# lars-frogner/Impact

Measured on AMD Instinct MI355X. Metric: voxels stepped/sec + remesh tris/sec, 512^3 grid, 1/2/4/8 MI355X, higher is better.
Workload: dtype i8 voxels, f32 SDF/mesh arithmetic, f64 moments; 1 GPU; config-2 SDF asteroid x2.05 -> 502^3 grid = 512^3 stored voxels (32768 chunks); parallelism=single GPU, voxels_per_gpu=134217728, regions=1, triangles=1813104

## Files before the change

### impact_amd/csrc/derive.hip

```cpp
#include "chunk_passes.hpp"
#include "table_roles.hpp"
#include "many.hpp"

#ifndef IVX_DERIVE_WAVES
#define IVX_DERIVE_WAVES 6
#endif

namespace {

struct DeriveParams {
    uint32_t cx, cy, cz;
};

__device__ __forceinline__ uint32_t row_mask(uint4 s) {
    uint32_t w[4] = {s.x, s.y, s.z, s.w};
    uint32_t m = 0;
#pragma unroll
    for (int q = 0; q < 4; ++q) m |= ((((w[q] >> 7) & 0x01010101u) * 0x00204081u >> 21) & 0xFu) << (4 * q);
    return m;
}

__device__ __forceinline__ uint32_t nbr_row_mask(const GridView& g, const ivx_chunk_info* info, size_t c, uint32_t off) {
    const uint32_t gen = info[c].gen_kind;
    const uint32_t rm = row_mask(*reinterpret_cast<const uint4*>(g.sdf + c * IVX_CHUNK_VOXELS + off));
// ... 465 lines not shown
            const bool only_empty = (cnt[0] | cnt[1] | cnt[2] | cnt[3] | cnt[4] | cnt[5]) == 0 && (ci_.flags & CF_ONLY_EMPTY);
            ci_.flags = (uint8_t)(ob | (only_empty ? CF_ONLY_EMPTY : 0u));
            uint32_t fd = 0;
#pragma unroll
            for (int f = 0; f < 6; ++f) fd |= own_fd[f] << (2 * f);
            ci_.face_dist = (uint16_t)fd;
            ci_.uniform_type = 0;
        } else if (kind == KIND_UNIFORM) {
            ci_.flags = 0;
            ci_.face_dist = 0x555;
            ci_.uniform_type = (uint8_t)utype;
        } else {
            ci_.flags = 0;
            ci_.face_dist = 0;
        }
        info[chunk] = ci_;
    }
    IVX_T(g, li, 5);
    }
}
template <bool SIGNS>
__global__ __launch_bounds__(256) __attribute__((amdgpu_waves_per_eu(IVX_DERIVE_WAVES, 8))) void k_derive(DeriveArgs a) {
    derive_body<SIGNS>(a, blockIdx.x, gridDim.x);
}
IVX_MANY_TWIN(k_derive_planes_many, DeriveArgs, derive_body<false>, __launch_bounds__(256) __attribute__((amdgpu_waves_per_eu(IVX_DERIVE_WAVES, 8))))
IVX_MANY_TWIN(k_derive_signs_many, DeriveArgs, derive_body<true>, __launch_bounds__(256) __attribute__((amdgpu_waves_per_eu(IVX_DERIVE_WAVES, 8))))
IVX_MANY_LAUNCHER(many_derive_planes, k_derive_planes_many, DeriveArgs, 256)
IVX_MANY_LAUNCHER(many_derive_signs, k_derive_signs_many, DeriveArgs, 256)

#ifndef IVX_DERIVE_FLOOD_CAP
#define IVX_DERIVE_FLOOD_CAP 32
#endif
#ifndef IVX_DERIVE_WAVE_WAVES
#define IVX_DERIVE_WAVE_WAVES 5
#endif

#ifdef IVX_WG_TRACE
#define IVX_TW(g, entry, slot)                                                                      \
    do {                                                                                            \
        if ((threadIdx.x & 63u) == 0u) (g).trace[(size_t)(entry) * 8 + (slot)] = wall_clock64();    \
    } while (0)
#else
#define IVX_TW(g, entry, slot) \
    do {                       \
    } while (0)
#endif

__device__ __forceinline__ void ivx_wave_lds_sync() {
    __builtin_amdgcn_fence(__ATOMIC_SEQ_CST, "workgroup");
    __builtin_amdgcn_wave_barrier();
}
__device__ __forceinline__ uint32_t ivx_run_fill_up(uint32_t m, uint32_t x) { return m & (((m + x) ^ m) | x); }
__device__ __forceinline__ uint32_t ivx_run_fill(uint32_t m, uint32_t x) {
    x &= m;
    return ivx_run_fill_up(m, x) | __builtin_bitreverse32(ivx_run_fill_up(__builtin_bitreverse32(m), __builtin_bitreverse32(x)));
}
__device__ __forceinline__ uint32_t ivx_dpp_u32_shr1(uint32_t v) { return (uint32_t)__builtin_amdgcn_update_dpp(0, (int)v, 0x111, 0xF, 0xF, true); }
__device__ __forceinline__ uint32_t ivx_dpp_u32_shl1(uint32_t v) { return (uint32_t)__builtin_amdgcn_update_dpp(0, (int)v, 0x101, 0xF, 0xF, true); }
__device__ __forceinline__ uint32_t ivx_wave_or(uint32_t v) {
    v |= (uint32_t)__builtin_amdgcn_update_dpp(0, (int)v, 0x111, 0xF, 0xF, true);
    v |= (uint32_t)__builtin_amdgcn_update_dpp(0, (int)v, 0x112, 0xF, 0xF, true);
    v |= (uint32_t)__builtin_amdgcn_update_dpp(0, (int)v, 0x114, 0xF, 0xF, true);
    v |= (uint32_t)__builtin_amdgcn_update_dpp(0, (int)v, 0x118, 0xF, 0xF, true);
    return ((uint32_t)__builtin_amdgcn_readlane((int)v, 15) | (uint32_t)__builtin_amdgcn_readlane((int)v, 31)) |
           ((uint32_t)__builtin_amdgcn_readlane((int)v, 47) | (uint32_t)__builtin_amdgcn_readlane((int)v, 63));
}

// ... 20 lines not shown
            G |= q > 0 ? F[q > 0 ? q - 1 : 0] : (a > 0u ? up : 0u);
            G |= q < 3 ? F[q < 3 ? q + 1 : 3] : (a < 3u ? dn : 0u);
            N[q] = ivx_run_fill(M[q], G);
            miss = miss || N[q] != M[q];
            grew = grew || N[q] != F[q];
        }
        if (!__ballot(miss)) return 1u;
        if (!__ballot(grew)) return 0u;
#pragma unroll
        for (int q = 0; q < 4; ++q) F[q] = N[q];
    }
    return 0u;
}

__device__ __forceinline__ void moments_rows_wave(double D, double Dz1, double Dz2, double (*s_red)[10], uint32_t i, uint32_t j, int gi, int gj) {
    const double I = (double)gi, J = (double)gj;
    const double qx = 2.0 * I + 1.0, qy = 2.0 * J + 1.0;
    const double cx = 3.0 * I * I + 3.0 * I + 1.0, cy = 3.0 * J * J + 3.0 * J + 1.0;
    const double r0 = ivx_row16_sum_f64(D), r1 = ivx_row16_sum_f64(D * qy), r2 = ivx_row16_sum_f64(D * cy);
    const double r3 = ivx_row16_sum_f64(Dz1), r4 = ivx_row16_sum_f64(qy * Dz1), r5 = ivx_row16_sum_f64(Dz2);
    if (j == 15u) {
        double* o = s_red[i];
        o[0] = r0;
        o[1] = r0 * qx;
        o[2] = r1;
        o[3] = r3;
        o[4] = r2 + r5;
        o[5] = r0 * cx + r5;
        o[6] = r0 * cx + r2;
        o[7] = r1 * qx;
        o[8] = r4;
        o[9] = r3 * qx;
    }
}

__device__ __forceinline__ void derive_wave_body(const DeriveArgs& a_) {
    const GridView& g = a_.g;
    uint8_t* __restrict__ flags_out = a_.flags_out;
    int8_t* __restrict__ sdf_rw = a_.sdf_rw;
    uint8_t* __restrict__ type_rw = a_.type_rw;
    ivx_chunk_info* __restrict__ info = a_.info;
    uint16_t* __restrict__ signs = a_.signs;
    uint8_t* __restrict__ kface_out = a_.kface_out;
    uint32_t* __restrict__ active_list = a_.active_list;
    const uint32_t* __restrict__ list_in = a_.list_in;
    const DeriveFused& fz = a_.fz;
    __shared__ float s_dens[256];
    __shared__ uint16_t s_mtab[256];
    __shared__ uint16_t s_occ[4][18 * 18 + 4];
    __shared__ double s_red_all[4][16][10];
    const uint32_t tid = threadIdx.x, lane = tid & 63u;
    const uint32_t wave = (uint32_t)__builtin_amdgcn_readfirstlane((int)(tid >> 6));
    uint16_t* occ = s_occ[wave];
    double (*s_red)[10] = s_red_all[wave];
    if (fz.parts & IVX_PART_MOMENTS) s_dens[tid] = fz.dens[tid], s_mtab[tid] = moments_table_entry(tid);
    __syncthreads();
    const uint32_t la = lane >> 4, j = lane & 15u;
    const uint32_t n_active = a_.work_counts[0];
    const uint32_t n_walk = gridDim.x * 4u;
    const uint32_t sx = g.cy * g.cz;
    const uint32_t* sw = reinterpret_cast<const uint32_t*>(g.signs);
    for (uint32_t li = ivx_xcd_remap(blockIdx.x, gridDim.x) * 4u + wave; li < n_active; li += n_walk) {
    IVX_TW(g, li, 0);
    const uint32_t chunk = IVX_LIST_CHUNK(list_in[li]);
    const int ck = chunk % g.cz, cj = (chunk / g.cz) % g.cy, ci = chunk / sx;
    const size_t base = (size_t)chunk * IVX_CHUNK_VOXELS;
    const bool has_zlo = ck > 0, has_zhi = ck + 1 < (int)g.cz;
    const size_t c_lo = has_zlo ? (size_t)chunk - 1 : (size_t)chunk, c_hi = has_zhi ? (size_t)chunk + 1 : (size_t)chunk;
    const uint32_t nf = la, nr = j;
    bool n_present;
    size_t nc;
    uint32_t noff;
    if (nf == 0) n_present = ci > 0, nc = (size_t)chunk - sx, noff = 240u + nr;
    else if (nf == 1) n_present = ci + 1 < (int)g.cx, nc = (size_t)chunk + sx, noff = nr;
    else if (nf == 2) n_present = cj > 0, nc = (size_t)chunk - g.cz, noff = nr * 16u + 15u;
    else n_present = cj + 1 < (int)g.cy, nc = (size_t)chunk + g.cz, noff = nr * 16u;
    if (!n_present) nc = chunk;
    uint2 own_rec = reinterpret_cast<const uint2*>(info)[chunk];
    uint32_t gen_lo = reinterpret_cast<const uint32_t*>(info)[2 * c_lo], gen_hi = reinterpret_cast<const uint32_t*>(info)[2 * c_hi];
    uint32_t ngen = reinterpret_cast<const uint32_t*>(info)[2 * nc];
    uint32_t type0 = *reinterpret_cast<const uint32_t*>(g.type + base);
    uint32_t nrow = sw[(nc * 256 + noff) >> 1];
    uint32_t ow[4], bl[4], bh[4];
#pragma unroll
    for (int q = 0; q < 4; ++q) {
        const uint32_t r = (4u * la + q) * 16u + j;
        ow[q] = sw[((size_t)chunk * 256 + r) >> 1];
        bl[q] = sw[(c_lo * 256 + r) >> 1];
        bh[q] = sw[(c_hi * 256 + r) >> 1];
    }
    asm volatile("" : "+v"(own_rec.x), "+v"(own_rec.y), "+v"(gen_lo), "+v"(gen_hi), "+v"(ngen), "+v"(type0), "+v"(nrow));
    asm volatile("" : "+v"(ow[0]), "+v"(ow[1]), "+v"(ow[2]), "+v"(ow[3]), "+v"(bl[0]), "+v"(bl[1]), "+v"(bl[2]), "+v"(bl[3]));
    asm volatile("" : "+v"(bh[0]), "+v"(bh[1]), "+v"(bh[2]), "+v"(bh[3]));
    own_rec.x = (uint32_t)__builtin_amdgcn_readfirstlane((int)own_rec.x), own_rec.y = (uint32_t)__builtin_amdgcn_readfirstlane((int)own_rec.y);
    gen_lo = ((uint32_t)__builtin_amdgcn_readfirstlane((int)gen_lo) >> 8) & 0xFFu, gen_hi = ((uint32_t)__builtin_amdgcn_readfirstlane((int)gen_hi) >> 8) & 0xFFu;
    type0 = (uint32_t)__builtin_amdgcn_readfirstlane((int)type0);
    ngen = (ngen >> 8) & 0xFFu;
    ivx_chunk_info own_info;
    own_info.kind = (uint8_t)(own_rec.x & 0xFFu);
    own_info.gen_kind = (uint8_t)((own_rec.x >> 8) & 0xFFu);
    own_info.flags = (uint8_t)((own_rec.x >> 16) & 0xFFu);
    own_info.uniform_type = (uint8_t)(own_rec.x >> 24);
    own_info.face_dist = (uint16_t)(own_rec.y & 0xFFFFu);
    own_info.region_count = (uint8_t)((own_rec.y >> 16) & 0xFFu);
    own_info.boundary_region_count = (uint8_t)(own_rec.y >> 24);
    const uint32_t gen = own_info.gen_kind;
    const bool own_uniform = gen == KIND_UNIFORM;
    uint32_t m[4], zl = 0u, zh = 0u;
    const uint32_t half = 16u * (j & 1u);
#pragma unroll
    for (int q = 0; q < 4; ++q) {
        m[q] = own_uniform ? 0xFFFFu : (gen == KIND_VOID ? 0u : ((ow[q] >> half) & 0xFFFFu));
        const uint32_t lo = (bl[q] >> half >> 15) & 1u, hi = (bh[q] >> half) & 1u;
        if (has_zlo && (gen_lo == KIND_NONUNIFORM ? lo : (gen_lo == KIND_UNIFORM ? 1u : 0u))) zl |= 1u << q;
        if (has_zhi && (gen_hi == KIND_NONUNIFORM ? hi : (gen_hi == KIND_UNIFORM ? 1u : 0u))) zh |= 1u << q;
        occ[(4u * la + q + 1u) * 18u + j + 1u] = (uint16_t)m[q];
    }
    uint32_t nm = 0u;
    {
        const uint32_t nrow_odd = nf == 2 ? 1u : (nf == 3 ? 0u : (nr & 1u));
        const uint32_t rm = (nrow >> (16u * nrow_odd)) & 0xFFFFu;
        if (n_present) nm = ngen == KIND_NONUNIFORM ? rm : (ngen == KIND_UNIFORM ? 0xFFFFu : 0u);
        if (nf == 0) occ[0 * 18 + nr + 1] = (uint16_t)nm;
        else if (nf == 1) occ[17 * 18 + nr + 1] = (uint16_t)nm;
        else if (nf == 2) occ[(nr + 1) * 18 + 0] = (uint16_t)nm;
        else occ[(nr + 1) * 18 + 17] = (uint16_t)nm;
    }
    uint32_t cnt[12];
    {
        const uint32_t p0 = __popc(m[0]), p3 = __popc(m[3]), pc = (p0 + __popc(m[1])) + (__popc(m[2]) + p3);
        cnt[0] = (uint32_t)__builtin_amdgcn_readlane((int)ivx_row16_sum(p0), 15);
        cnt[1] = (uint32_t)__builtin_amdgcn_readlane((int)ivx_row16_sum(p3), 63);
        cnt[2] = ((uint32_t)__builtin_amdgcn_readlane((int)pc, 0) + (uint32_t)__builtin_amdgcn_readlane((int)pc, 16)) +
                 ((uint32_t)__builtin_amdgcn_readlane((int)pc, 32) + (uint32_t)__builtin_amdgcn_readlane((int)pc, 48));
        cnt[3] = ((uint32_t)__builtin_amdgcn_readlane((int)pc, 15) + (uint32_t)__builtin_amdgcn_readlane((int)pc, 31)) +
                 ((uint32_t)__builtin_amdgcn_readlane((int)pc, 47) + (uint32_t)__builtin_amdgcn_readlane((int)pc, 63));
        uint32_t z0 = 0, z1 = 0, nz0 = 0, nz1 = 0;
#pragma unroll
        for (int q = 0; q < 4; ++q) {
            z0 += (uint32_t)__popcll(__ballot((m[q] & 1u) != 0u));
            z1 += (uint32_t)__popcll(__ballot(((m[q] >> 15) & 1u) != 0u));
            nz0 += (uint32_t)__popcll(__ballot(((zl >> q) & 1u) != 0u));
            nz1 += (uint32_t)__popcll(__ballot(((zh >> q) & 1u) != 0u));
        }
        cnt[4] = z0, cnt[5] = z1, cnt[10] = nz0, cnt[11] = nz1;
        const uint32_t nfs = ivx_row16_sum(__popc(nm));
        cnt[6] = (uint32_t)__builtin_amdgcn_readlane((int)nfs, 15), cnt[7] = (uint32_t)__builtin_amdgcn_readlane((int)nfs, 31);
        cnt[8] = (uint32_t)__builtin_amdgcn_readlane((int)nfs, 47), cnt[9] = (uint32_t)__builtin_amdgcn_readlane((int)nfs, 63);
    }
    {
        uint32_t bi = 0, bjw = 0;
#pragma unroll
        for (int q = 0; q < 4; ++q) {
            const unsigned long long b = __ballot(m[q] != 0u);
#pragma unroll
            for (int s = 0; s < 4; ++s)
                if ((b >> (16 * s)) & 0xFFFFull) bi |= 1u << (4 * s + q);
            bjw |= (uint32_t)b | (uint32_t)(b >> 32);
        }
        const uint32_t bj = (bjw | (bjw >> 16)) & 0xFFFFu;
        const uint32_t ku = ivx_wave_or((m[0] | m[1]) | (m[2] | m[3]));
        uint32_t packed = 0;
        if (bi) {
            packed = 0x80000000u | (uint32_t)(__ffs(bi) - 1) | ((uint32_t)(31 - __clz(bi)) << 4) | ((uint32_t)(__ffs(bj) - 1) << 8) |
                     ((uint32_t)(31 - __clz(bj)) << 12) | ((uint32_t)(__ffs(ku) - 1) << 16) | ((uint32_t)(31 - __clz(ku)) << 20);
        }
        if (lane == 0u && IVX_DBG_KEEP(64u)) a_.bbox[chunk] = packed;
    }
    IVX_TW(g, li, 1);
    uint32_t own_fd[6], nbr_full = 0, own_mixed = 0;
#pragma unroll
    for (int f = 0; f < 6; ++f) {
        const uint32_t c = cnt[f];
        own_fd[f] = c == 0 ? FD_EMPTY : (c == 256 ? FD_FULL : FD_MIXED);
        if (own_fd[f] == FD_MIXED) own_mixed |= 1u << f;
        if (cnt[6 + f] == 256) nbr_full |= 1u << f;
    }
    uint32_t kind = gen;
    if (gen == KIND_UNIFORM && nbr_full != 0x3Fu) kind = KIND_NONUNIFORM;
    const uint32_t utype = own_uniform ? (own_info.kind == KIND_NONUNIFORM ? (type0 & 0xFFu) : (uint32_t)own_info.uniform_type) : 0u;
    const bool fresh = own_uniform && own_info.kind != KIND_NONUNIFORM;
    const uint32_t quirk = own_mixed & nbr_full;
    ivx_wave_lds_sync();
    IVX_TW(g, li, 2);
    bool t_x = false, t_y = false, t_z = false;
#pragma unroll
    for (int q = 0; q < 4; ++q) {
        const uint32_t i = 4u * la + q, r = i * 16u + j;
        const uint32_t xdn = occ[i * 18u + j + 1u], xup = occ[(i + 2u) * 18u + j + 1u];
        const uint32_t ydn = occ[(i + 1u) * 18u + j], yup = occ[(i + 1u) * 18u + j + 2u];
        const uint32_t mq = m[q], zlo = (zl >> q) & 1u, zhi = (zh >> q) & 1u;
        t_x = t_x || (i == 15u && (mq & xup) != 0u);
        t_y = t_y || (j == 15u && (mq & yup) != 0u);
        t_z = t_z || ((((mq >> 15) & 1u) & zhi) != 0u);
        if (kind != KIND_NONUNIFORM) continue;
        const uint32_t zdn = (mq << 1) | zlo, zup = (mq >> 1) | (zhi << 15);
        const uint32_t e = ~mq & 0xFFFFu;
        uint32_t dm[6];
        dm[0] = (mq & xdn) | ((i == 0u && (quirk & 1u)) ? e : 0u);
        dm[1] = (mq & ydn) | ((j == 0u && (quirk & 4u)) ? e : 0u);
// ... 57 lines not shown
            }
            all_full = !__ballot(not_full);
            any = __ballot(nonempty) != 0ull;
            touches = __ballot(on_edge) != 0ull;
            const bool several_runs = __ballot(runs2) != 0ull;
            const uint32_t lack_all = ivx_wave_or(lack);
            if (any && !all_full && !several_runs && (~lack_all & 0xFFFFu) != 0u) {
                uint32_t b[16];
#pragma unroll
                for (int q = 0; q < 4; ++q) {
                    const unsigned long long bq = __ballot(R[q] != 0u);
#pragma unroll
                    for (int s = 0; s < 4; ++s) b[4 * s + q] = (uint32_t)(bq >> (16 * s)) & 0xFFFFu;
                }
                bool ok = true;
                uint32_t lines = 0u;
#pragma unroll
                for (int i = 0; i < 16; ++i) {
                    const uint32_t bn = i < 15 ? b[i < 15 ? i + 1 : 15] : 0u, runs = b[i] & ~(b[i] << 1);
                    ok = ok && (b[i] == 0u || ((runs & (runs - 1u)) == 0u && (bn == 0u || (b[i] & bn) != 0u)));
                    if (b[i]) lines |= 1u << i;
                }
                const uint32_t line_runs = lines & ~(lines << 1);
                slab = ok && (line_runs & (line_runs - 1u)) == 0u;
            }
        }
        if (!any || all_full) {
            const uint32_t lab = any ? 0u : 0xFFFFFFFFu;
            if (kind == KIND_NONUNIFORM && IVX_DBG_KEEP(8u)) {
#pragma unroll
                for (int q = 0; q < 4; ++q)
                    *reinterpret_cast<uint4*>(fz.labels + base + (size_t)((4u * la + q) * 16u + j) * 16) = make_uint4(lab, lab, lab, lab);
            }
            if (lane == 0u) rp[0] = any ? chunk * 256u : NODE_NONE;
            rc = any ? 1u : 0u;
            brc = any ? 1u : 0u;
        } else if (slab || ivx_flood_connected(R, lane)) {
#pragma unroll
            for (int q = 0; q < 4; ++q) {
                uint32_t w[4] = {0, 0, 0, 0};
#pragma unroll
                for (int k = 0; k < 16; ++k)
                    if (!((R[q] >> k) & 1u)) w[k >> 2] |= 0xFFu << (8 * (k & 3));
                if (IVX_DBG_KEEP(8u)) *reinterpret_cast<uint4*>(fz.labels + base + (size_t)((4u * la + q) * 16u + j) * 16) = make_uint4(w[0], w[1], w[2], w[3]);
            }
            if (lane == 0u) rp[0] = chunk * 256u;
            rc = 1u;
            brc = touches ? 1u : 0u;
        } else {
            if (lane == 0u) fz.multi_list[atomicAdd(&fz.rscalar[2], 1u)] = chunk;
            rc = 2u;
            brc = 0u;
        }
    }
    IVX_TW(g, li, 4);
    if ((fz.parts & IVX_PART_MOMENTS) && kind == KIND_NONUNIFORM && IVX_DBG_KEEP(16u)) {
        const uint32_t type = fresh ? utype : a_.signs_type;
#pragma unroll
        for (int q = 0; q < 4; ++q) {
            const uint32_t i = 4u * la + q;
            double D, Dz1, Dz2;
            moments_row_sums_one_type(m[q], type, s_dens, s_mtab, ck * 16, D, Dz1, Dz2);
            moments_rows_wave(D, Dz1, Dz2, s_red, i, j, (ci + (int)fz.x_off) * 16 + (int)i, cj * 16 + (int)j);
        }
        ivx_wave_lds_sync();
        if (lane < 10u) {
            double t = s_red[0][lane];
#pragma unroll
            for (int r = 1; r < 16; ++r) t += s_red[r][lane];
            fz.chunk_moments[(size_t)chunk * 10 + lane] = t;
        }
    }
    if (lane == 0u && IVX_DBG_KEEP(32u)) {
        a_.touch[chunk] = (uint8_t)tb;
        const bool obscured = kind == KIND_NONUNIFORM && nbr_full == 0x3Fu;
        active_list[li] = chunk | (kind << 24) | (gen << 26) | ((kind == KIND_NONUNIFORM && !obscured) ? (1u << 28) : 0u);
        ivx_chunk_info ci_ = own_info;
        ci_.kind = (uint8_t)kind;
        ci_.region_count = (uint8_t)rc;
        ci_.boundary_region_count = (uint8_t)brc;
        if (kind == KIND_NONUNIFORM) {
            uint32_t ob = 0;
#pragma unroll
            for (int f = 0; f < 6; ++f)
                if ((nbr_full >> f) & 1u) ob |= 1u << ((f & 1) * 3 + (f >> 1));
            const bool only_empty = (cnt[0] | cnt[1] | cnt[2] | cnt[3] | cnt[4] | cnt[5]) == 0 && (ci_.flags & CF_ONLY_EMPTY);
            ci_.flags = (uint8_t)(ob | (only_empty ? CF_ONLY_EMPTY : 0u));
            uint32_t fd = 0;
#pragma unroll
            for (int f = 0; f < 6; ++f) fd |= own_fd[f] << (2 * f);
            ci_.face_dist = (uint16_t)fd;
            ci_.uniform_type = 0;
        } else if (kind == KIND_UNIFORM) {
            ci_.flags = 0;
            ci_.face_dist = 0x555;
            ci_.uniform_type = (uint8_t)utype;
        } else {
            ci_.flags = 0;
            ci_.face_dist = 0;
        }
        info[chunk] = ci_;
    }
    IVX_TW(g, li, 5);
    ivx_wave_lds_sync();
    }
}
__global__ __launch_bounds__(256) __attribute__((amdgpu_waves_per_eu(IVX_DERIVE_WAVE_WAVES, 8))) void k_derive_wave(DeriveArgs a) { derive_wave_body(a); }

struct ListRebuildArgs {
    GridView g;
    const ivx_chunk_info* info;
    uint32_t* work_counts;
    uint32_t* next_work_count;
    uint32_t* active_list;
    uint32_t* mesh_counts;
};
__device__ __forceinline__ void list_rebuild_body(const ListRebuildArgs& a, uint32_t bid, uint32_t) {
    const GridView& g = a.g;
    const ivx_chunk_info* __restrict__ info = a.info;
    uint32_t* __restrict__ work_counts = a.work_counts;
    uint32_t* __restrict__ next_work_count = a.next_work_count;
    uint32_t* __restrict__ active_list = a.active_list;
    uint32_t* __restrict__ mesh_counts = a.mesh_counts;
    __shared__ uint32_t s_w[4];
    __shared__ uint32_t s_base;
    const uint32_t tid = threadIdx.x, lane = tid & 63u, wave = tid >> 6;
    if (bid == 0 && tid == 0) next_work_count[0] = 0u;
    const uint32_t n_chunks = g.cx * g.cy * g.cz;
    const uint32_t chunk = bid * 256u + tid;
    const bool live = chunk < n_chunks;
    bool settled = false;
    uint32_t entry = 0;
    if (live) {
        const ivx_chunk_info own = info[chunk];
        const uint32_t gen = own.gen_kind;
        settled = gen == KIND_VOID;
        if (gen == KIND_UNIFORM) {
// ... 115 lines not shown
    return IVX_OK;
}

ivx_roles::PresetArgs ivx_preset_args(ivx_grid* g, uint32_t groups) {
    const uint32_t n_groups = (g->n_chunks + 255u) / 256u;
    ivx_roles::PresetArgs a;
    a.groups = groups;
    a.rscalar = g->rscalar;
    a.sn_sums = g->group_sums + n_groups;
    a.n_sn = IVX_SN_GROUP_WORDS * n_groups;
    a.eval_count = g->samp_len ? g->samp_len + g->n_chunks : nullptr;
    return a;
}

int ivx_launch_step_preset(ivx_grid* g, uint32_t groups) {
    if (!groups) return IVX_OK;
    const ivx_roles::PresetArgs a = ivx_preset_args(g, groups);
    IVX_KLAUNCH(k_step_preset, dim3((a.n_sn + 255u) / 256u), dim3(256), 0, g->ctx->stream, a);
    IVX_HIP_CHECK(hipGetLastError());
    g->scratch_dirty &= ~groups;
    return IVX_OK;
}

#ifdef IVX_DERIVE_DEBUG
static void derive_debug_mask() {
    static bool done = false;
    if (done) return;
    done = true;
    const char* e = getenv("IVX_DERIVE_SKIP");
    const uint32_t v = e ? (uint32_t)strtoul(e, nullptr, 0) : 0u;
    (void)hipMemcpyToSymbol(HIP_SYMBOL(ivx_dbg_derive_skip), &v, sizeof(v));
}
#endif
int ivx_launch_derive(ivx_grid* g, uint32_t parts, uint32_t preset_groups) {
#ifdef IVX_DERIVE_DEBUG
    derive_debug_mask();
#endif
    GridView v = ivx_view(g);
    DeriveFused fz;
    fz.parts = parts;
    fz.x_off = g->x_off;
    fz.labels = g->llabel;
    fz.rparent = g->rparent;
    fz.rscalar = g->rscalar;
    fz.multi_list = g->ccl_scratch;
    fz.dens = g->dens_dev;
    fz.chunk_moments = g->chunk_moments;
    if ((parts & IVX_PART_REGIONS) && !(preset_groups & IVX_SCRATCH_REGIONS) && (g->scratch_dirty & IVX_SCRATCH_REGIONS))
        IVX_HIP_CHECK(ivx_memset_async(g->rscalar, 0, 16 * sizeof(uint32_t), g->ctx->stream));
    if (parts & IVX_PART_REGIONS) g->scratch_dirty |= IVX_SCRATCH_REGIONS;
    g->bbox_valid = 1;
    uint32_t* next_count = ivx_wc(g);
    g->wc_cur ^= 1u;
    const uint32_t roll = ((g->scratch_dirty & IVX_SCRATCH_EVAL) && g->samp_len) ? IVX_SCRATCH_EVAL_ROLL : 0u;
    ChunkPreArgs face_settle;
    {
        ChunkPreArgs pa;
        memset(&pa, 0, sizeof(pa));
        pa.g = v, pa.info = g->info, pa.bbox = g->chunk_bbox, pa.mesh_counts = g->chunk_counts, pa.chunk_class = g->chunk_class, pa.touch = g->chunk_touch;
        pa.rparent = g->rparent, pa.work_counts = ivx_wc(g), pa.next_work_count = next_count, pa.active_list = g->active_list;
        pa.preset = ivx_preset_args(g, preset_groups | roll);
        if (g->ghost_event && g->ghost_split && ivx_has_interior_planes(g)) pa.defer_ghost = 1u;
        const uint32_t blocks = (g->n_chunks + 255u) / 256u;
        if (!ivx_many_try(g->ctx, g, IVX_MK_CHUNK_PRE, blocks, pa)) IVX_KLAUNCH(k_chunk_pre, dim3(blocks), dim3(256), 0, g->ctx->stream, pa);
        face_settle = pa;
    }
    g->scratch_dirty &= ~preset_groups;
    if (roll) g->scratch_dirty &= ~IVX_SCRATCH_EVAL;
    uint32_t derive_grid = ivx_list_grid(g);
    if (g->last_active) {
        const uint32_t per_round = (uint32_t)g->ctx->n_cu * 32u;
        const uint32_t each = (g->last_active + per_round / 2u) / per_round > 1u ? (g->last_active + per_round / 2u) / per_round : 1u;
        derive_grid = (g->last_active + each - 1u) / each;
        const uint32_t lo = (g->n_chunks + 255u) / 256u;
        if (derive_grid < lo) derive_grid = lo;
    }
    DeriveArgs da = derive_args(g, v, fz);
    if (g->signs_current) da.signs_type = (uint32_t)g->signs_type;
    uint32_t wave_grid;
    {
        const uint32_t per_round = (uint32_t)g->ctx->n_cu * 4u * IVX_DERIVE_WAVE_WAVES;
        const uint32_t n = g->last_active ? g->last_active : per_round;
        const uint32_t each = (n + per_round / 2u) / per_round > 1u ? (n + per_round / 2u) / per_round : 1u;
        wave_grid = ((n + each - 1u) / each + 3u) / 4u;
    }
    auto sweep = [&](uint32_t x_part) {
        da.x_part = x_part;
        if (g->signs_current) {
            if (ivx_many_try(g->ctx, g, IVX_MK_DERIVE_SIGNS, derive_grid, da)) return;
            if (x_part == IVX_XPART_ALL && v.ghost_sdf[0] == nullptr && v.ghost_sdf[1] == nullptr)
                IVX_KLAUNCH(k_derive_wave, dim3(wave_grid), dim3(256), 0, g->ctx->stream, da);
            else
                IVX_KLAUNCH(k_derive<true>, dim3(derive_grid), dim3(256), 0, g->ctx->stream, da);
        } else {
            if (!ivx_many_try(g->ctx, g, IVX_MK_DERIVE_PLANES, derive_grid, da)) IVX_KLAUNCH(k_derive<false>, dim3(derive_grid), dim3(256), 0, g->ctx->stream, da);
        }
    };
    if (g->ghost_event) {
        const bool interior = g->ghost_split && ivx_has_interior_planes(g);
        if (interior) sweep(IVX_XPART_INTERIOR);
        (void)ivx_many_break();
        static const bool skip_wait = getenv("IVX_DEBUG_SKIP_GHOST_WAIT") && atoi(getenv("IVX_DEBUG_SKIP_GHOST_WAIT")) == 1;
        if (!skip_wait) IVX_HIP_CHECK(hipStreamWaitEvent(g->ctx->stream, static_cast<hipEvent_t>(g->ghost_event), 0));
        g->ghost_event = nullptr;
        if (face_settle.defer_ghost) IVX_KLAUNCH(k_face_settle, dim3((2u * g->cc[1] * g->cc[2] + 255u) / 256u), dim3(256), 0, g->ctx->stream, face_settle);
        sweep(interior ? IVX_XPART_FACES : IVX_XPART_ALL);
    } else {
        sweep(IVX_XPART_ALL);
    }
    g->active_list_stale = 0;
    g->planes_compact = 1;
    IVX_HIP_CHECK(hipGetLastError());
    return IVX_OK;
}

int ivx_launch_derive_box(ivx_grid* g, uint32_t parts, const uint32_t lo[3], const uint32_t cc[3], uint32_t* d_out_list) {
    GridView v = ivx_view(g);
// ... 65 lines not shown
```

### impact_amd/csrc/ivx_api.hip

```cpp
#include <algorithm>
#include <array>
#include <functional>
#include <cmath>
#include <atomic>
#include <chrono>
#include <cstring>
#include <limits>
#include <map>
#include <unordered_map>
#include <new>
#include <vector>

#include <type_traits>

#include <dlfcn.h>

#include "ivx_host.hpp"

static thread_local char g_error[512] = "";

void ivx_set_error(const char* fmt, ...) {
    va_list ap;
    va_start(ap, fmt);
    vsnprintf(g_error, sizeof(g_error), fmt, ap);
// ... 587 lines not shown

int ivx_grid_stage_counters(ivx_grid* g, uint32_t out[4]) {
    IVX_REQUIRE(g && out, IVX_ERR_INVALID, "ivx_grid_stage_counters: null argument");
    for (int i = 0; i < 4; ++i) out[i] = 0;
    int rc;
    if (g->samp_len) {
        uint32_t ev[3];
        if ((rc = d2h(g, ev, g->samp_len + g->n_chunks + ((g->scratch_dirty & IVX_SCRATCH_EVAL) ? 0 : 8), sizeof(ev)))) return rc;
        out[0] = ev[0] + ev[1] + ev[2];
    }
    if ((rc = d2h(g, &out[1], g->rscalar + 2, sizeof(uint32_t)))) return rc;
    if ((rc = d2h(g, &out[2], g->chunk_offsets + 2 * (size_t)g->n_chunks + 2, sizeof(uint32_t)))) return rc;
    out[3] = g->n_chunks;
    return IVX_OK;
}

void* ivx_grid_device_ptr(ivx_grid* g, int which) {
    if (!g) return nullptr;
    if (which >= 0 && which < 4 && ivx_ensure_dense(g) != IVX_OK) return nullptr;
    if (which == 0 || which == 1 || which == 4) ivx_planes_touched(g);
    switch (which) {
        case 0: return g->sdf;
        case 1: return g->type;
        case 2: return g->flags;
        case 3: return g->llabel;
        case 4: return g->info;
        case 5: return g->rparent;
#ifdef IVX_WG_TRACE
        case 6: return g->chunk_moments;
#endif
        case 7: return g->samp_len;
        case 8: return g->samp_ops;
        case 10: return g->sn_hard;
        case 9: return ivx_sn_hard_count(g);
        default: return nullptr;
    }
}

int ivx_sdf_sample(ivx_grid* g, const ivx_sdf_processed_node* nodes, size_t n_nodes, uint32_t stack_size, const uint32_t grid_shape[3],
                   const float shifted_grid_center[3], uint8_t voxel_type) {
    IVX_REQUIRE(g && grid_shape && shifted_grid_center, IVX_ERR_INVALID, "ivx_sdf_sample: null argument");
    IVX_REQUIRE(n_nodes == 0 || nodes, IVX_ERR_INVALID, "ivx_sdf_sample: null node array");
    for (int d = 0; d < 3; ++d) {
        const uint32_t cap = (d == 0 ? g->gx : g->cc[d]) * 16u;
        IVX_REQUIRE(grid_shape[d] <= cap, IVX_ERR_INVALID, "ivx_sdf_sample: grid shape %u exceeds the chunk grid (%u voxels) along axis %d", grid_shape[d], cap, d);
    }
    int depth = 0, max_depth = 0;
    for (size_t i = 0; i < n_nodes; ++i) {
        const uint32_t k = nodes[i].kind;
        IVX_REQUIRE(k <= 9, IVX_ERR_INVALID, "ivx_sdf_sample: unsupported node kind %u", k);
        IVX_REQUIRE(k != 6 || nodes[i].reserved[1] <= 255u, IVX_ERR_INVALID, "ivx_sdf_sample: noise node with more than 255 octaves");
        if (k <= 2) max_depth = std::max(max_depth, ++depth);
        else if (k >= 7) {
            IVX_REQUIRE(depth >= 2, IVX_ERR_INVALID, "ivx_sdf_sample: malformed node program (combination without two operands)");
            --depth;
        } else if (k == 5 || k == 6) {
            IVX_REQUIRE(depth >= 1, IVX_ERR_INVALID, "ivx_sdf_sample: malformed node program (scaling / noise without operand)");
        }
    }
    IVX_REQUIRE(n_nodes == 0 || depth == 1, IVX_ERR_INVALID, "ivx_sdf_sample: malformed node program (final stack depth %d)", depth);
    IVX_REQUIRE((uint32_t)max_depth <= stack_size || n_nodes == 0, IVX_ERR_INVALID, "ivx_sdf_sample: stack_size %u < required %d", stack_size, max_depth);
    int rc;
    if ((rc = ensure_dev_scratch(g, std::max<size_t>(n_nodes, 1) * sizeof(ivx_sdf_processed_node)))) return rc;
    {
        std::vector<ivx_sdf_processed_node> annotated(nodes, nodes + n_nodes);
        ivx_sdf_annotate_host(annotated.data(), n_nodes);
// ... 1986 lines not shown
```

### impact_amd/csrc/ivx_internal.hpp

```cpp
#pragma once
#include <hip/hip_runtime.h>

#include <cstdarg>
#include <cstdint>
#include <cstdio>
#include <cstring>

#include "../../include/impact_voxel_hip.h"
#include "many.hpp"

static inline hipError_t ivx_memset_async(void* p, int v, size_t n, hipStream_t s) {
    (void)ivx_many_break();
    return hipMemsetAsync(p, v, n, s);
}
static inline hipError_t ivx_memcpy_async(void* d, const void* src, size_t n, hipMemcpyKind k, hipStream_t s) {
    (void)ivx_many_break();
    return hipMemcpyAsync(d, src, n, k, s);
}
static inline hipError_t ivx_stream_sync(hipStream_t s) {
    (void)ivx_many_break();
    return hipStreamSynchronize(s);
}
static inline hipError_t ivx_memcpy_sync(void* d, const void* src, size_t n, hipMemcpyKind k) {
    (void)ivx_many_break();
// ... 11 lines not shown
#define VF_EMPTY 0x01u
#define VF_X_DN 0x04u
#define VF_Y_DN 0x08u
#define VF_Z_DN 0x10u
#define VF_X_UP 0x20u
#define VF_Y_UP 0x40u
#define VF_Z_UP 0x80u
#define CF_ONLY_EMPTY 0x40u
#define CF_FULLY_OBSCURED 0x3Fu
#define KIND_VOID 0
#define KIND_UNIFORM 1
#define KIND_NONUNIFORM 2
#define FD_EMPTY 0
#define FD_FULL 1
#define FD_MIXED 2
#define TYPE_DUMMY 255
#define SD_VOID_LIMIT 100

struct ivx_buf {
    void* p = nullptr;
    size_t bytes = 0;
};
struct ivx_mapped {
    void* p = nullptr;
    void* dev = nullptr;
    size_t bytes = 0;
};

struct ivx_ctx {
    int device;
    hipStream_t stream;
    bool own_stream;
    int n_cu;
    ivx_mapped pinned_scratch;
    ivx_buf dev_scratch;
    hipStream_t aux_stream;
    void* many_recorder;
    int many_error;
    ivx_buf drag_scratch;
    void* cull_state;
    void* bvol_state;
};

struct ivx_block {
    void* dev;
    void* pinned;
    int refs;
};

struct ivx_grid {
    ivx_ctx* ctx;
    uint32_t cc[3];
    uint32_t n_chunks;
    size_t n_vox;
    float extent;
    uint32_t x_off, gx;
    char* arena;
    ivx_block* arena_block;
    ivx_block* host_block;
    int8_t* sdf;
    uint8_t* type;
    uint8_t* flags;
    uint8_t* llabel;
    ivx_chunk_info* info;
    uint32_t* chunk_bbox;
    int8_t* ghost_sdf[2];
// ... 244 lines not shown
    const uint8_t* kface;
#ifdef IVX_WG_TRACE
    unsigned long long* trace;
#endif
    const int8_t* ghost_sdf[2];
    const uint8_t* ghost_type[2];
    const ivx_chunk_info* info;
    const ivx_chunk_info* ghost_info[2];
};

#define IVX_XPART_ALL 0u
#define IVX_XPART_INTERIOR 1u
#define IVX_XPART_FACES 2u
#ifdef __HIPCC__
__device__ __forceinline__ bool ivx_xpart_skip(const GridView& g, uint32_t x_part, uint32_t ci) {
    if (x_part == IVX_XPART_ALL) return false;
    const bool face = (ci == 0u && g.ghost_sdf[0] != nullptr) || (ci + 1u == g.cx && g.ghost_sdf[1] != nullptr);
    return face != (x_part == IVX_XPART_FACES);
}
#endif

#define IVX_LIST_CHUNK(w) ((w) & 0xFFFFFFu)
#define IVX_LIST_KIND(w) (((w) >> 24) & 3u)
#define IVX_LIST_GEN(w) (((w) >> 26) & 3u)
#define IVX_LIST_EXPOSED(w) (((w) >> 28) & 1u)

static inline uint32_t ivx_list_grid(const ivx_grid* g) {
    uint32_t n = g->last_active ? g->last_active + g->last_active / 8u + 64u : (uint32_t)g->ctx->n_cu * 32u;
    const uint32_t lo = (g->n_chunks + 255u) / 256u;
    if (n > g->n_chunks) n = g->n_chunks;
    return n < lo ? lo : n;
}

static inline bool ivx_has_interior_planes(const ivx_grid* g) { return (int)g->cc[0] - (g->has_ghost[0] ? 1 : 0) - (g->has_ghost[1] ? 1 : 0) > 0; }
static inline uint32_t* ivx_wc(const ivx_grid* g) { return g->work_counts + g->wc_cur; }
static inline void ivx_planes_touched(ivx_grid* g) {
    g->signs_current = 0;
    g->needs_current = 0;
}
#define IVX_SCRATCH_EVAL_ROLL 8u
#define IVX_SCRATCH_REGIONS 1u
#define IVX_SCRATCH_SN 2u
#define IVX_SN_TAIL_WORDS 288u
#define IVX_SN_GROUP_WORDS 32u
#define IVX_SCRATCH_EVAL 4u

static inline GridView ivx_view(const ivx_grid* g) {
    GridView v;
    v.cx = g->cc[0];
    v.cy = g->cc[1];
    v.cz = g->cc[2];
    v.sdf = g->sdf;
    v.type = g->type;
    v.signs = g->chunk_signs;
    v.kface = g->kface;
#ifdef IVX_WG_TRACE
    v.trace = reinterpret_cast<unsigned long long*>(g->chunk_moments);
#endif
    v.info = g->info;
    for (int s = 0; s < 2; ++s) {
        if (g->has_ghost[s] && g->ghost_ext[s]) {
            const size_t cols = (size_t)g->cc[1] * g->cc[2];
            v.ghost_sdf[s] = reinterpret_cast<const int8_t*>(g->ghost_ext[s]);
            v.ghost_type[s] = g->ghost_ext[s] + cols * 256;
            v.ghost_info[s] = reinterpret_cast<const ivx_chunk_info*>(g->ghost_ext[s] + cols * 512);
        } else {
// ... 85 lines not shown
```

Baseline: 841.2 billion voxels/s.

## Prefetch next chunk's rows in derive wave loop and size grid by occupancy

The per-wave derive loop now issues the global loads for the next list entry (info records, sign rows, neighbour row) partway through processing the current chunk, so memory latency overlaps with compute. The grid size is now computed from the queried resident occupancy instead of a fixed waves-per-EU constant, which is raised from 5 to 6, and an env override is added. The empty-label mask expansion becomes a multiply-based bit spread, and a sched barrier is added in the moments loop. These changes add register pressure from carrying a second row set, which may limit occupancy.

```diff
diff --git a/impact_amd/csrc/derive.hip b/impact_amd/csrc/derive.hip
--- a/impact_amd/csrc/derive.hip
+++ b/impact_amd/csrc/derive.hip
@@ -521,7 +521,7 @@
 #define IVX_DERIVE_FLOOD_CAP 32
 #endif
 #ifndef IVX_DERIVE_WAVE_WAVES
-#define IVX_DERIVE_WAVE_WAVES 5
+#define IVX_DERIVE_WAVE_WAVES 6
 #endif
 
 #ifdef IVX_WG_TRACE
@@ -608,6 +608,49 @@
         o[8] = r4;
         o[9] = r3 * qx;
     }
+}
+
+struct DeriveWaveRows {
+    uint32_t chunk, next_word;
+    uint2 own_rec;
+    uint32_t gen_lo, gen_hi, ngen, type0, nrow, ow[4], bl[4], bh[4];
+};
+__device__ __forceinline__ void derive_wave_fetch(const GridView& g, const ivx_chunk_info* info, const uint32_t* list_in, uint32_t chunk, uint32_t next_at,
+                                                  uint32_t lane, DeriveWaveRows& w) {
+    asm volatile("" : "+v"(lane));
+    const uint32_t la = lane >> 4, j = lane & 15u;
+    const uint32_t sx = g.cy * g.cz;
+    const uint32_t* sw = reinterpret_cast<const uint32_t*>(g.signs);
+    const int ck = chunk % g.cz, cj = (chunk / g.cz) % g.cy, ci = chunk / sx;
+    const size_t c_lo = ck > 0 ? (size_t)chunk - 1 : (size_t)chunk, c_hi = ck + 1 < (int)g.cz ? (size_t)chunk + 1 : (size_t)chunk;
+    const uint32_t nf = la, nr = j;
+    bool n_present;
+    size_t nc;
+    uint32_t noff;
+    if (nf == 0) n_present = ci > 0, nc = (size_t)chunk - sx, noff = 240u + nr;
+    else if (nf == 1) n_present = ci + 1 < (int)g.cx, nc = (size_t)chunk + sx, noff = nr;
+    else if (nf == 2) n_present = cj > 0, nc = (size_t)chunk - g.cz, noff = nr * 16u + 15u;
+    else n_present = cj + 1 < (int)g.cy, nc = (size_t)chunk + g.cz, noff = nr * 16u;
+    if (!n_present) nc = chunk;
+    w.chunk = chunk;
+    w.next_word = list_in[next_at];
+    w.own_rec = reinterpret_cast<const uint2*>(info)[chunk];
+    w.gen_lo = reinterpret_cast<const uint32_t*>(info)[2 * c_lo], w.gen_hi = reinterpret_cast<const uint32_t*>(info)[2 * c_hi];
+    w.ngen = reinterpret_cast<const uint32_t*>(info)[2 * nc];
+    w.type0 = *reinterpret_cast<const uint32_t*>(g.type + (size_t)chunk * IVX_CHUNK_VOXELS);
+    w.nrow = sw[(nc * 256 + noff) >> 1];
+#pragma unroll
+    for (int q = 0; q < 4; ++q) {
+        const uint32_t r = (4u * la + q) * 16u + j;
+        w.ow[q] = sw[((size_t)chunk * 256 + r) >> 1];
+        w.bl[q] = sw[(c_lo * 256 + r) >> 1];
+        w.bh[q] = sw[(c_hi * 256 + r) >> 1];
+    }
+}
+__device__ __forceinline__ void derive_wave_pin(DeriveWaveRows& w) {
+    asm volatile("" : "+v"(w.own_rec.x), "+v"(w.own_rec.y), "+v"(w.gen_lo), "+v"(w.gen_hi), "+v"(w.ngen), "+v"(w.type0), "+v"(w.nrow), "+v"(w.next_word));
+    asm volatile("" : "+v"(w.ow[0]), "+v"(w.ow[1]), "+v"(w.ow[2]), "+v"(w.ow[3]), "+v"(w.bl[0]), "+v"(w.bl[1]), "+v"(w.bl[2]), "+v"(w.bl[3]));
+    asm volatile("" : "+v"(w.bh[0]), "+v"(w.bh[1]), "+v"(w.bh[2]), "+v"(w.bh[3]));
 }
 
 __device__ __forceinline__ void derive_wave_body(const DeriveArgs& a_) {
@@ -629,45 +672,41 @@
     const uint32_t wave = (uint32_t)__builtin_amdgcn_readfirstlane((int)(tid >> 6));
     uint16_t* occ = s_occ[wave];
     double (*s_red)[10] = s_red_all[wave];
-    if (fz.parts & IVX_PART_MOMENTS) s_dens[tid] = fz.dens[tid], s_mtab[tid] = moments_table_entry(tid);
-    __syncthreads();
-    const uint32_t la = lane >> 4, j = lane & 15u;
     const uint32_t n_active = a_.work_counts[0];
     const uint32_t n_walk = gridDim.x * 4u;
     const uint32_t sx = g.cy * g.cz;
-    const uint32_t* sw = reinterpret_cast<const uint32_t*>(g.signs);
-    for (uint32_t li = ivx_xcd_remap(blockIdx.x, gridDim.x) * 4u + wave; li < n_active; li += n_walk) {
-    IVX_TW(g, li, 0);
-    const uint32_t chunk = IVX_LIST_CHUNK(list_in[li]);
+    uint32_t li = ivx_xcd_remap(blockIdx.x, gridDim.x) * 4u + wave;
+    float dens_t = 0.0f;
+    if (fz.parts & IVX_PART_MOMENTS) dens_t = fz.dens[tid];
+    DeriveWaveRows rows;
+    {
+        const bool have = li < n_active;
+        const uint32_t word = list_in[have ? li : 0u];
+        if (have) IVX_TW(g, li, 0);
+        derive_wave_fetch(g, info, list_in, have ? IVX_LIST_CHUNK(word) : 0u, li + n_walk < n_active ? li + n_walk : 0u, lane, rows);
+    }
+    if (fz.parts & IVX_PART_MOMENTS) s_dens[tid] = dens_t, s_mtab[tid] = moments_table_entry(tid);
+    __syncthreads();
+    while (li < n_active) {
+    uint32_t lane_e = lane;
+    asm volatile("" : "+v"(lane_e));
+    const uint32_t la = lane_e >> 4, j = lane_e & 15u;
+    const uint32_t chunk = rows.chunk;
     const int ck = chunk % g.cz, cj = (chunk / g.cz) % g.cy, ci = chunk / sx;
     const size_t base = (size_t)chunk * IVX_CHUNK_VOXELS;
     const bool has_zlo = ck > 0, has_zhi = ck + 1 < (int)g.cz;
-    const size_t c_lo = has_zlo ? (size_t)chunk - 1 : (size_t)chunk, c_hi = has_zhi ? (size_t)chunk + 1 : (size_t)chunk;
     const uint32_t nf = la, nr = j;
-    bool n_present;
-    size_t nc;
-    uint32_t noff;
-    if (nf == 0) n_present = ci > 0, nc = (size_t)chunk - sx, noff = 240u + nr;
-    else if (nf == 1) n_present = ci + 1 < (int)g.cx, nc = (size_t)chunk + sx, noff = nr;
-    else if (nf == 2) n_present = cj > 0, nc = (size_t)chunk - g.cz, noff = nr * 16u + 15u;
-    else n_present = cj + 1 < (int)g.cy, nc = (size_t)chunk + g.cz, noff = nr * 16u;
-    if (!n_present) nc = chunk;
-    uint2 own_rec = reinterpret_cast<const uint2*>(info)[chunk];
-    uint32_t gen_lo = reinterpret_cast<const uint32_t*>(info)[2 * c_lo], gen_hi = reinterpret_cast<const uint32_t*>(info)[2 * c_hi];
-    uint32_t ngen = reinterpret_cast<const uint32_t*>(info)[2 * nc];
-    uint32_t type0 = *reinterpret_cast<const uint32_t*>(g.type + base);
-    uint32_t nrow = sw[(nc * 256 + noff) >> 1];
+    const bool n_present = nf == 0 ? ci > 0 : (nf == 1 ? ci + 1 < (int)g.cx : (nf == 2 ? cj > 0 : cj + 1 < (int)g.cy));
+    const uint32_t li_next = li + n_walk;
+    const bool has_next = li_next < n_active;
+    derive_wave_pin(rows);
+    const uint32_t next_chunk = IVX_LIST_CHUNK((uint32_t)__builtin_amdgcn_readfirstlane((int)rows.next_word));
+    uint2 own_rec = rows.own_rec;
+    uint32_t gen_lo = rows.gen_lo, gen_hi = rows.gen_hi, ngen = rows.ngen, type0 = rows.type0;
+    const uint32_t nrow = rows.nrow;
     uint32_t ow[4], bl[4], bh[4];
 #pragma unroll
-    for (int q = 0; q < 4; ++q) {
-        const uint32_t r = (4u * la + q) * 16u + j;
-        ow[q] = sw[((size_t)chunk * 256 + r) >> 1];
-        bl[q] = sw[(c_lo * 256 + r) >> 1];
-        bh[q] = sw[(c_hi * 256 + r) >> 1];
-    }
-    asm volatile("" : "+v"(own_rec.x), "+v"(own_rec.y), "+v"(gen_lo), "+v"(gen_hi), "+v"(ngen), "+v"(type0), "+v"(nrow));
-    asm volatile("" : "+v"(ow[0]), "+v"(ow[1]), "+v"(ow[2]), "+v"(ow[3]), "+v"(bl[0]), "+v"(bl[1]), "+v"(bl[2]), "+v"(bl[3]));
-    asm volatile("" : "+v"(bh[0]), "+v"(bh[1]), "+v"(bh[2]), "+v"(bh[3]));
+    for (int q = 0; q < 4; ++q) ow[q] = rows.ow[q], bl[q] = rows.bl[q], bh[q] = rows.bh[q];
     own_rec.x = (uint32_t)__builtin_amdgcn_readfirstlane((int)own_rec.x), own_rec.y = (uint32_t)__builtin_amdgcn_readfirstlane((int)own_rec.y);
     gen_lo = ((uint32_t)__builtin_amdgcn_readfirstlane((int)gen_lo) >> 8) & 0xFFu, gen_hi = ((uint32_t)__builtin_amdgcn_readfirstlane((int)gen_hi) >> 8) & 0xFFu;
     type0 = (uint32_t)__builtin_amdgcn_readfirstlane((int)type0);
@@ -702,6 +741,11 @@
         else if (nf == 2) occ[(nr + 1) * 18 + 0] = (uint16_t)nm;
         else occ[(nr + 1) * 18 + 17] = (uint16_t)nm;
     }
+    DeriveWaveRows next_rows;
+    if (has_next) {
+        IVX_TW(g, li_next, 0);
+        derive_wave_fetch(g, info, list_in, next_chunk, li_next + n_walk < n_active ? li_next + n_walk : 0u, lane, next_rows);
+    }
     uint32_t cnt[12];
     {
         const uint32_t p0 = __popc(m[0]), p3 = __popc(m[3]), pc = (p0 + __popc(m[1])) + (__popc(m[2]) + p3);
@@ -741,7 +785,7 @@
             packed = 0x80000000u | (uint32_t)(__ffs(bi) - 1) | ((uint32_t)(31 - __clz(bi)) << 4) | ((uint32_t)(__ffs(bj) - 1) << 8) |
                      ((uint32_t)(31 - __clz(bj)) << 12) | ((uint32_t)(__ffs(ku) - 1) << 16) | ((uint32_t)(31 - __clz(ku)) << 20);
         }
-        if (lane == 0u && IVX_DBG_KEEP(64u)) a_.bbox[chunk] = packed;
+        if (lane_e == 0u && IVX_DBG_KEEP(64u)) a_.bbox[chunk] = packed;
     }
     IVX_TW(g, li, 1);
     uint32_t own_fd[6], nbr_full = 0, own_mixed = 0;
@@ -865,23 +909,26 @@
                 for (int q = 0; q < 4; ++q)
                     *reinterpret_cast<uint4*>(fz.labels + base + (size_t)((4u * la + q) * 16u + j) * 16) = make_uint4(lab, lab, lab, lab);
             }
-            if (lane == 0u) rp[0] = any ? chunk * 256u : NODE_NONE;
+            if (lane_e == 0u) rp[0] = any ? chunk * 256u : NODE_NONE;
             rc = any ? 1u : 0u;
             brc = any ? 1u : 0u;
-        } else if (slab || ivx_flood_connected(R, lane)) {
+        } else if (slab || ivx_flood_connected(R, lane_e)) {
 #pragma unroll
             for (int q = 0; q < 4; ++q) {
-                uint32_t w[4] = {0, 0, 0, 0};
-#pragma unroll
-                for (int k = 0; k < 16; ++k)
-                    if (!((R[q] >> k) & 1u)) w[k >> 2] |= 0xFFu << (8 * (k & 3));
+                const uint32_t empty = ~R[q] & 0xFFFFu;
+                uint32_t w[4];
+#pragma unroll
+                for (int h = 0; h < 4; ++h) {
+                    const uint32_t s = __umul24((empty >> (4 * h)) & 0xFu, 0x00204081u) & 0x01010101u;
+                    w[h] = (s << 8) - s;
+                }
                 if (IVX_DBG_KEEP(8u)) *reinterpret_cast<uint4*>(fz.labels + base + (size_t)((4u * la + q) * 16u + j) * 16) = make_uint4(w[0], w[1], w[2], w[3]);
             }
-            if (lane == 0u) rp[0] = chunk * 256u;
+            if (lane_e == 0u) rp[0] = chunk * 256u;
             rc = 1u;
             brc = touches ? 1u : 0u;
         } else {
-            if (lane == 0u) fz.multi_list[atomicAdd(&fz.rscalar[2], 1u)] = chunk;
+            if (lane_e == 0u) fz.multi_list[atomicAdd(&fz.rscalar[2], 1u)] = chunk;
             rc = 2u;
             brc = 0u;
         }
@@ -895,16 +942,17 @@
             double D, Dz1, Dz2;
             moments_row_sums_one_type(m[q], type, s_dens, s_mtab, ck * 16, D, Dz1, Dz2);
             moments_rows_wave(D, Dz1, Dz2, s_red, i, j, (ci + (int)fz.x_off) * 16 + (int)i, cj * 16 + (int)j);
+            __builtin_amdgcn_sched_barrier(0);
         }
         ivx_wave_lds_sync();
-        if (lane < 10u) {
-            double t = s_red[0][lane];
-#pragma unroll
-            for (int r = 1; r < 16; ++r) t += s_red[r][lane];
-            fz.chunk_moments[(size_t)chunk * 10 + lane] = t;
-        }
-    }
-    if (lane == 0u && IVX_DBG_KEEP(32u)) {
+        if (lane_e < 10u) {
+            double t = s_red[0][lane_e];
+#pragma unroll
+            for (int r = 1; r < 16; ++r) t += s_red[r][lane_e];
+            fz.chunk_moments[(size_t)chunk * 10 + lane_e] = t;
+        }
+    }
+    if (lane_e == 0u && IVX_DBG_KEEP(32u)) {
         a_.touch[chunk] = (uint8_t)tb;
         const bool obscured = kind == KIND_NONUNIFORM && nbr_full == 0x3Fu;
         active_list[li] = chunk | (kind << 24) | (gen << 26) | ((kind == KIND_NONUNIFORM && !obscured) ? (1u << 28) : 0u);
@@ -936,6 +984,9 @@
     }
     IVX_TW(g, li, 5);
     ivx_wave_lds_sync();
+    if (!has_next) break;
+    rows = next_rows;
+    li = li_next;
     }
 }
 __global__ __launch_bounds__(256) __attribute__((amdgpu_waves_per_eu(IVX_DERIVE_WAVE_WAVES, 8))) void k_derive_wave(DeriveArgs a) { derive_wave_body(a); }
@@ -1117,6 +1168,26 @@
     (void)hipMemcpyToSymbol(HIP_SYMBOL(ivx_dbg_derive_skip), &v, sizeof(v));
 }
 #endif
+static uint32_t derive_wave_resident(ivx_ctx* c) {
+    if (!c->derive_wave_resident) {
+        int per_cu = 0;
+        if (hipOccupancyMaxActiveBlocksPerMultiprocessor(&per_cu, k_derive_wave, 256, 0) != hipSuccess || per_cu < 1) {
+            (void)hipGetLastError();
+            per_cu = 1;
+        }
+        if (per_cu > IVX_DERIVE_WAVE_WAVES) per_cu = IVX_DERIVE_WAVE_WAVES;
+        c->derive_wave_resident = (uint32_t)c->n_cu * 4u * (uint32_t)per_cu;
+    }
+    return c->derive_wave_resident;
+}
+static uint32_t derive_wave_grid_override() {
+    static const uint32_t forced = [] {
+        const char* e = getenv("IVX_DERIVE_WAVE_GRID");
+        const unsigned long v = e ? strtoul(e, nullptr, 10) : 0ul;
+        return (uint32_t)(v > 65535ul ? 65535ul : v);
+    }();
+    return forced;
+}
 int ivx_launch_derive(ivx_grid* g, uint32_t parts, uint32_t preset_groups) {
 #ifdef IVX_DERIVE_DEBUG
     derive_debug_mask();
@@ -1164,10 +1235,9 @@
     if (g->signs_current) da.signs_type = (uint32_t)g->signs_type;
     uint32_t wave_grid;
     {
-        const uint32_t per_round = (uint32_t)g->ctx->n_cu * 4u * IVX_DERIVE_WAVE_WAVES;
-        const uint32_t n = g->last_active ? g->last_active : per_round;
-        const uint32_t each = (n + per_round / 2u) / per_round > 1u ? (n + per_round / 2u) / per_round : 1u;
-        wave_grid = ((n + each - 1u) / each + 3u) / 4u;
+        const uint32_t resident = derive_wave_resident(g->ctx);
+        wave_grid = ivx_wave_walk_grid(g->last_active ? g->last_active : resident, resident).workgroups;
+        if (const uint32_t forced = derive_wave_grid_override()) wave_grid = forced;
     }
     auto sweep = [&](uint32_t x_part) {
         da.x_part = x_part;
diff --git a/impact_amd/csrc/ivx_api.hip b/impact_amd/csrc/ivx_api.hip
--- a/impact_amd/csrc/ivx_api.hip
+++ b/impact_amd/csrc/ivx_api.hip
@@ -643,6 +643,8 @@
         case 7: return g->samp_len;
         case 8: return g->samp_ops;
         case 10: return g->sn_hard;
+        case 11: return g->chunk_bbox;
+        case 12: return g->chunk_touch;
         case 9: return ivx_sn_hard_count(g);
         default: return nullptr;
     }
diff --git a/impact_amd/csrc/ivx_internal.hpp b/impact_amd/csrc/ivx_internal.hpp
--- a/impact_amd/csrc/ivx_internal.hpp
+++ b/impact_amd/csrc/ivx_internal.hpp
@@ -67,6 +67,7 @@
     hipStream_t stream;
     bool own_stream;
     int n_cu;
+    uint32_t derive_wave_resident;
     ivx_mapped pinned_scratch;
     ivx_buf dev_scratch;
     hipStream_t aux_stream;
@@ -377,6 +378,19 @@
     return n < lo ? lo : n;
 }
 
+struct ivx_wave_walk {
+    uint32_t each;
+    uint32_t workgroups;
+};
+static inline ivx_wave_walk ivx_wave_walk_grid(uint32_t entries, uint32_t resident_waves) {
+    if (entries == 0u) entries = 1u;
+    if (resident_waves == 0u) resident_waves = 1u;
+    ivx_wave_walk w;
+    w.each = (entries + resident_waves - 1u) / resident_waves;
+    w.workgroups = ((entries + w.each - 1u) / w.each + 3u) / 4u;
+    return w;
+}
+
 static inline bool ivx_has_interior_planes(const ivx_grid* g) { return (int)g->cc[0] - (g->has_ghost[0] ? 1 : 0) - (g->has_ghost[1] ? 1 : 0) > 0; }
 static inline uint32_t* ivx_wc(const ivx_grid* g) { return g->work_counts + g->wc_cur; }
 static inline void ivx_planes_touched(ivx_grid* g) {
```

New measurement: 848.0 billion voxels/s, median of 2. No clear change (+0.8%).
